# karltan0328/POPE

Measured on AMD Instinct MI355X. Metric: image-pairs/s (DINOv2-S/14 extract+match, 640x480), higher is better.
Workload: dtype f16x3 (fp32 operands split hi+lo into f16, 3 MFMAs per product, fp32 accumulate)

## Files before the change

pope_amd/csrc/attention_f16x3.hip:

```cpp
#include "attention_common.h"
#include "kernels.h"
#include <type_traits>

namespace {
using namespace pope_attn;

typedef __attribute__((address_space(3))) s16x4* lds_s16x4_ptr;

constexpr int WAVES = 8;
constexpr int QB = 32 * WAVES;
constexpr int NT = 64 * WAVES;
constexpr int K_PLANE = KT * KST + 32, V_PLANE = KT * VST + 32;
constexpr size_t X3_ATTN_EPI_BYTES = size_t(32) * WAVES * OST * sizeof(float);

__device__ __forceinline__ void split4(f32x4 v, f16x4& hi, f16x4& lo) { pope_split4(v, hi, lo); }

#ifdef ATTN_STAMPS
__device__ unsigned long long g_attn_dbg[32 * 8];
#define ATTN_STAMP(t, slot)                                                                                     \
    do {                                                                                                        \
        if (blockIdx.x == 300 && tid == 0 && (t) < 32) g_attn_dbg[(t) * 8 + (slot)] = __builtin_readcyclecounter(); \
    } while (0)
#else
#define ATTN_STAMP(t, slot) do {} while (0)
#endif
__device__ unsigned long long g_attn_exact_passes;
constexpr int STAGE_H = 2 * (K_PLANE + V_PLANE);
constexpr size_t X3_ATTN_PIPE_BYTES = size_t(3) * STAGE_H * sizeof(_Float16);
static_assert(X3_ATTN_PIPE_BYTES >= X3_ATTN_EPI_BYTES, "epilogue staging fits the stages");

template <bool OUT_PLANES, bool IN_PLANES, bool DIAG = false>
__global__ __launch_bounds__(NT, 2) void attn_f16x3_pipe_kernel(const float* __restrict__ qkv, float* __restrict__ out,
                                                                  int N, int heads) {
    extern __shared__ __attribute__((aligned(16))) float smem[];
    _Float16* lds = reinterpret_cast<_Float16*>(smem);

    const int tid = threadIdx.x, lane = tid & 63, wave = tid >> 6;
    const int r = lane & 31, h = lane >> 5;
    const Block blk = decode_block(N, heads, QB);
    const int head = blk.head, b = blk.b, q0 = blk.q0;
    const int D = heads * HD, rs = 3 * D;
    const float* base = qkv + size_t(b) * N * rs;
    const int koff = D + head * HD;

    constexpr float QSCALE = 0.125f * 1.44269504088896340736f * (IN_PLANES ? 0.125f * 0.125f : 1.0f);
    f16x8 qh[4], ql[4];
    {
        const int qrow = q0 + wave * 32 + r;
#pragma unroll
        for (int kg = 0; kg < 4; ++kg) {
            f32x4 v0 = {0.f, 0.f, 0.f, 0.f}, v1 = {0.f, 0.f, 0.f, 0.f};
            if (qrow < N) {
                if constexpr (IN_PLANES) {
                    const _Float16* p = reinterpret_cast<const _Float16*>(base) + size_t(qrow) * 2 * rs +
                                        (head * 2 + (kg >> 1)) * 64 + 16 * (kg & 1) + 8 * h;
                    const f16x8 ph = *reinterpret_cast<const f16x8*>(p), pl = *reinterpret_cast<const f16x8*>(p + 32);
#pragma unroll
                    for (int e = 0; e < 4; ++e) {
                        v0[e] = float(ph[e]) + float(pl[e]);
                        v1[e] = float(ph[4 + e]) + float(pl[4 + e]);
                    }
                } else {
                    const float* p = base + size_t(qrow) * rs + head * HD + 16 * kg + 8 * h;
                    v0 = *reinterpret_cast<const f32x4*>(p);
                    v1 = *reinterpret_cast<const f32x4*>(p + 4);
                }
            }
            f16x4 h0, l0, h1, l1;
            split4(v0 * QSCALE, h0, l0);
            split4(v1 * QSCALE, h1, l1);
            qh[kg] = cat(h0, h1);
            ql[kg] = cat(l0, l1);
        }
    }

    const __amdgpu_buffer_rsrc_t rsrc =
        __builtin_amdgcn_make_buffer_rsrc(const_cast<float*>(base), 0, unsigned(N) * unsigned(rs) * 4u, 0x00020000);
    constexpr int RPP = NT / 16, NP = KT / RPP;
    const int srow = tid >> 4, scol = (tid & 15) * 4;
    unsigned kvoff[NP];
#pragma unroll
    for (int i = 0; i < NP; ++i) kvoff[i] = (unsigned(srow + RPP * i) * unsigned(rs) + scol + koff) * 4u;
    const unsigned tile_bytes = unsigned(KT) * unsigned(rs) * 4u, v_delta = unsigned(D) * 4u;
    f32x4 rk[NP], rv[NP];
    auto load_kv = [&](int kt) {
#pragma unroll
        for (int i = 0; i < NP; ++i) {
            rk[i] = __builtin_bit_cast(f32x4, __builtin_amdgcn_raw_buffer_load_b128(rsrc, kvoff[i], kt * tile_bytes, 0));
            rv[i] = __builtin_bit_cast(f32x4, __builtin_amdgcn_raw_buffer_load_b128(rsrc, kvoff[i] + v_delta, kt * tile_bytes, 0));
        }
    };
    f16x4 skh[NP], skl[NP], svh[NP], svl[NP];
    auto split_kv = [&]() {
#pragma unroll
        for (int i = 0; i < NP; ++i) {
            split4(rk[i], skh[i], skl[i]);
            split4(rv[i], svh[i], svl[i]);
        }
    };
    auto write_k_row = [&](int st, int i) {
        _Float16* S = lds + st * STAGE_H;
        *reinterpret_cast<f16x4*>(S + (srow + RPP * i) * KST + scol) = skh[i];
        *reinterpret_cast<f16x4*>(S + K_PLANE + (srow + RPP * i) * KST + scol) = skl[i];
    };
    auto write_v_row = [&](int st, int i) {
        _Float16* S = lds + st * STAGE_H;
        *reinterpret_cast<f16x4*>(S + 2 * K_PLANE + (srow + RPP * i) * VST + scol) = svh[i];
        *reinterpret_cast<f16x4*>(S + 2 * K_PLANE + V_PLANE + (srow + RPP * i) * VST + scol) = svl[i];
    };
    auto write_kv = [&](int st) {
        _Float16* S = lds + st * STAGE_H;
#pragma unroll
        for (int i = 0; i < NP; ++i) {
            *reinterpret_cast<f16x4*>(S + (srow + RPP * i) * KST + scol) = skh[i];
            *reinterpret_cast<f16x4*>(S + K_PLANE + (srow + RPP * i) * KST + scol) = skl[i];
            *reinterpret_cast<f16x4*>(S + 2 * K_PLANE + (srow + RPP * i) * VST + scol) = svh[i];
            *reinterpret_cast<f16x4*>(S + 2 * K_PLANE + V_PLANE + (srow + RPP * i) * VST + scol) = svl[i];
        }
    };

    typedef __attribute__((ext_vector_type(4))) unsigned u32x4;
    u32x4 pa[4] = {}, pb[4] = {};
    const int pkey = tid >> 3, pp = tid & 7;
    const unsigned pl_off = unsigned(pkey) * unsigned(rs) * 4u + unsigned((D >> 5) + head * 2) * 128u + unsigned(pp) * 16u;
    const unsigned pl_vdelta = unsigned(D >> 5) * 128u;
    auto load_planes = [&](int kt, u32x4 (&st)[4]) {
        if (kt * KT >= N) return;
#pragma unroll
        for (int c = 0; c < 4; ++c)
            st[c] = __builtin_amdgcn_raw_buffer_load_b128(rsrc, pl_off + (c >> 1) * pl_vdelta + (c & 1) * 128u, kt * tile_bytes, 0);
    };
    auto write_chunk = [&](int st, int c, const u32x4 (&regs)[4]) {
        _Float16* S = lds + st * STAGE_H + (c < 2 ? 0 : 2 * K_PLANE) + (pp >> 2) * (c < 2 ? K_PLANE : V_PLANE) +
                      pkey * (c < 2 ? KST : VST) + (c & 1) * 32 + (pp & 3) * 8;
        *reinterpret_cast<u32x4*>(S) = regs[c];
    };

    const int v_off = tr_off(lane, h);
    auto vfrag = [&](const _Float16* plane, int u, int s, int dt) {
        const _Float16* p = plane + v_off + (32 * u + 16 * s) * VST + 32 * dt;
        const s16x4 a = __builtin_amdgcn_ds_read_tr16_b64_v4i16((lds_s16x4_ptr)(p));
        const s16x4 c = __builtin_amdgcn_ds_read_tr16_b64_v4i16((lds_s16x4_ptr)(p + 8 * VST));
        return cat(__builtin_bit_cast(f16x4, a), __builtin_bit_cast(f16x4, c));
    };

    f32x16 o0, o1, sb[2][2];
    using P0 = std::integral_constant<int, 0>;
    using P1 = std::integral_constant<int, 1>;
#pragma unroll
    for (int i = 0; i < 16; ++i) { o0[i] = 0.f; o1[i] = 0.f; }
    f32x2 l_run = {0.f, 0.f};
    f32x16 nref;
#pragma unroll
    for (int i = 0; i < 16; ++i) nref[i] = INFINITY;

    struct KFrag { f16x8 k0h, k0l, k1h, k1l; };
    auto read_kfrag = [&](int st, int kg, KFrag& f) {
        const _Float16* kb_h = lds + st * STAGE_H + r * KST + 8 * h + 16 * kg;
        f.k0h = *reinterpret_cast<const f16x8*>(kb_h);
        f.k0l = *reinterpret_cast<const f16x8*>(kb_h + K_PLANE);
        f.k1h = *reinterpret_cast<const f16x8*>(kb_h + 32 * KST);
        f.k1l = *reinterpret_cast<const f16x8*>(kb_h + K_PLANE + 32 * KST);
    };
    auto qk_step = [&](int kg, int j, const KFrag& f, f32x16& d0, f32x16& d1, auto biased) {
        const f32x16 zero = {};
        const f32x16 c_init = decltype(biased)::value ? nref : zero;
        if (j == 0) d0 = mfma_f16(f.k0l, qh[kg], kg == 0 ? c_init : d0);
        if (j == 1) d1 = mfma_f16(f.k1l, qh[kg], kg == 0 ? c_init : d1);
        if (j == 2) d0 = mfma_f16(f.k0h, ql[kg], d0);
        if (j == 3) d1 = mfma_f16(f.k1h, ql[kg], d1);
        if (j == 4) d0 = mfma_f16(f.k0h, qh[kg], d0);
        if (j == 5) d1 = mfma_f16(f.k1h, qh[kg], d1);
    };
    constexpr float LAZY_HEADROOM = 8.0f, LAZY_LIMIT_LOG2 = 15.99f;
    f32x2 sm_ls = {0.f, 0.f};
    auto exact_prepare = [&](const f32x16& c0, const f32x16& c1) __attribute__((always_inline)) {
        float mt = vmax3(c0[0], c1[0], c0[1]);
#pragma unroll
        for (int i = 1; i < 15; ++i) mt = vmax3(mt, c1[i], c0[i + 1]);
        mt = __builtin_fmaxf(mt, c1[15]);
        float ma, mb;
        pope_xor32_pair(mt, ma, mb);
        const float ref_old = -nref[0];
        const float ref_new = __builtin_fmaxf(ref_old, __builtin_fmaxf(ma, mb) - LAZY_HEADROOM);
        const float delta = ref_old - ref_new;
        const float alpha = __builtin_amdgcn_exp2f(delta);
#pragma unroll
        for (int i = 0; i < 16; ++i) nref[i] = -ref_new;
        l_run = l_run * alpha;
#pragma unroll
        for (int e = 0; e < 16; ++e) { o0[e] *= alpha; o1[e] *= alpha; }
        return delta;
    };
    auto exp_pair = [&](int i, f32x16& c0, f32x16& c1, auto biased) __attribute__((always_inline)) {
        f32x16& c = i < 8 ? c0 : c1;
        const int e = 2 * (i & 7);
        if constexpr (decltype(biased)::value) {
            c[e] = __builtin_amdgcn_exp2f(c[e]);
            c[e + 1] = __builtin_amdgcn_exp2f(c[e + 1]);
        } else {
            c[e] = __builtin_amdgcn_exp2f(c[e] + nref[0]);
            c[e + 1] = __builtin_amdgcn_exp2f(c[e + 1] + nref[0]);
        }
        float a0 = sm_ls[0], a1 = sm_ls[1];
        a0 += c[e];
        asm volatile("" : "+v"(a0));
        a1 += c[e + 1];
        asm volatile("" : "+v"(a1));
        sm_ls = f32x2{a0, a1};
    };
    auto softmax_slice = [&](int slot, auto ptag) __attribute__((always_inline)) {
        if (slot == 0) sm_ls = f32x2{0.f, 0.f};
        if (slot % 3 != 2)
            exp_pair((slot / 3) * 2 + slot % 3, sb[decltype(ptag)::value][0], sb[decltype(ptag)::value][1], std::true_type{});
    };
    float la_mt = 0.f;
    auto lookahead_slice = [&](int slot, const f32x16& n0, const f32x16& n1) __attribute__((always_inline)) {
        if (slot == 0) la_mt = vmax3(n0[0], n1[0], n0[1]);
        else if (slot < 15) la_mt = vmax3(la_mt, n1[slot], n0[slot + 1]);
        else if (slot == 15) la_mt = __builtin_fmaxf(la_mt, n1[15]);
    };
    auto advance = [&](f32x16& n0, f32x16& n1) __attribute__((always_inline)) {
        if (__builtin_expect(__builtin_amdgcn_ballot_w64(!(la_mt < LAZY_LIMIT_LOG2)) != 0, 0)) {
            if constexpr (DIAG)
                if (lane == 0) (void)__hip_atomic_fetch_add(&g_attn_exact_passes, 1ull, __ATOMIC_RELAXED, __HIP_MEMORY_SCOPE_AGENT);
            float ma, mb;
            pope_xor32_pair(la_mt, ma, mb);
            const float over = __builtin_fmaxf(__builtin_fmaxf(ma, mb) - LAZY_HEADROOM, 0.f);
            const float delta = -over, alpha = __builtin_amdgcn_exp2f(delta);
            const float nr = nref[0] + delta;
#pragma unroll
            for (int i = 0; i < 16; ++i) nref[i] = nr;
            l_run = l_run * alpha;
#pragma unroll
            for (int e = 0; e < 16; ++e) { o0[e] *= alpha; o1[e] *= alpha; }
#pragma unroll
            for (int i = 0; i < 16; ++i) { n0[i] += delta; n1[i] += delta; }
        }
    };
    auto settle = [&]() __attribute__((always_inline)) { l_run += sm_ls; };
    auto phase1 = [&](int st_next, auto ptag) {
        f32x16& n0 = sb[decltype(ptag)::value ^ 1][0];
        f32x16& n1 = sb[decltype(ptag)::value ^ 1][1];
        KFrag kf[2];
        read_kfrag(st_next, 0, kf[0]);
#pragma unroll
        for (int i = 0; i < 24; ++i) {
            const int kg = i / 6, j = i % 6;
            if (j == 0 && kg < 3) read_kfrag(st_next, kg + 1, kf[(kg + 1) & 1]);
            qk_step(kg, j, kf[kg & 1], n0, n1, std::true_type{});
            softmax_slice(i, ptag);
            __builtin_amdgcn_sched_barrier(0);
        }
    };
    auto softmax_only = [&](auto ptag) {
#pragma unroll
        for (int i = 0; i < 24; ++i) softmax_slice(i, ptag);
    };
    auto split_group = [&](int g, int half, f16x4& hi, f16x4& lo, auto ptag) {
        const int u = g >> 1, s2 = g & 1;
        f32x4 pv4;
#pragma unroll
        for (int e = 0; e < 4; ++e) pv4[e] = sb[decltype(ptag)::value][u][8 * s2 + 4 * half + e];
        split4(pv4, hi, lo);
    };
    auto phase2 = [&](int st, int st_write, auto split_tag, const u32x4 (&pregs)[4], auto ptag, auto look_tag) {
        constexpr bool SPLIT_KV = decltype(split_tag)::value;
        constexpr bool LOOK = decltype(look_tag)::value;
        const _Float16* Vh = lds + st * STAGE_H + 2 * K_PLANE;
        const _Float16* Vl = Vh + V_PLANE;
        f16x4 h0[2], l0[2], h1[2], l1[2];
        f16x8 vh[2][2], vl[2];
        split_group(0, 0, h0[0], l0[0], ptag);
        split_group(0, 1, h1[0], l1[0], ptag);
        vh[0][0] = vfrag(Vh, 0, 0, 0); vl[0] = vfrag(Vl, 0, 0, 0);
        vh[0][1] = vfrag(Vh, 0, 0, 1); vl[1] = vfrag(Vl, 0, 0, 1);
        __builtin_amdgcn_sched_barrier(0);
#pragma unroll
        for (int i = 0; i < 24; ++i) {
            const int g = i / 6, j = i % 6, cur = g & 1, nxt = cur ^ 1;
            const int u = (g + 1) >> 1, s2 = (g + 1) & 1;
            if (j == 0 && g < 3) { vh[nxt][0] = vfrag(Vh, u, s2, 0); vh[nxt][1] = vfrag(Vh, u, s2, 1); }
            const f16x8 ph = cat(h0[cur], h1[cur]), pl = cat(l0[cur], l1[cur]);
            if (j == 0) o0 = mfma_f16(vl[0], ph, o0);
            if (j == 1) o1 = mfma_f16(vl[1], ph, o1);
            if (j == 2) o0 = mfma_f16(vh[cur][0], pl, o0);
            if (j == 3) o1 = mfma_f16(vh[cur][1], pl, o1);
            if (j == 4) o0 = mfma_f16(vh[cur][0], ph, o0);
            if (j == 5) o1 = mfma_f16(vh[cur][1], ph, o1);
            if (j == 2 && g < 3) { vl[0] = vfrag(Vl, u, s2, 0); vl[1] = vfrag(Vl, u, s2, 1); }
            if (g < 3) {
                if (j == 1) split_group(g + 1, 0, h0[nxt], l0[nxt], ptag);
                if (j == 3) split_group(g + 1, 1, h1[nxt], l1[nxt], ptag);
            }
            if (LOOK && i % 3 != 1) lookahead_slice(i - (i + 1) / 3, sb[decltype(ptag)::value ^ 1][0], sb[decltype(ptag)::value ^ 1][1]);
            if (SPLIT_KV && j == 5) {
                if constexpr (IN_PLANES) {
                    write_chunk(st_write, g, pregs);
                } else {
                    const int i2 = g >> 1;
                    if (g & 1) { split4(rv[i2], svh[i2], svl[i2]); write_v_row(st_write, i2); }
                    else { split4(rk[i2], skh[i2], skl[i2]); write_k_row(st_write, i2); }
                }
            }
            __builtin_amdgcn_sched_barrier(0);
        }
    };

    const int nkt = (N + KT - 1) / KT;
    if constexpr (IN_PLANES) {
        load_planes(0, pa);
        load_planes(1, pb);
#pragma unroll
        for (int c = 0; c < 4; ++c) write_chunk(0, c, pa);
        load_planes(2, pa);
    } else {
        load_kv(0);
        split_kv();
        write_kv(0);
        if (nkt > 1) load_kv(1);
    }
    __syncthreads();
    {
        KFrag kf;
#pragma unroll
        for (int kg = 0; kg < 4; ++kg) {
            read_kfrag(0, kg, kf);
#pragma unroll
            for (int j = 0; j < 6; ++j) qk_step(kg, j, kf, sb[0][0], sb[0][1], std::false_type{});
        }
    }
    if (nkt == 1) mask_tail(0, h, N, sb[0][0], sb[0][1]);
    if constexpr (IN_PLANES) {
#pragma unroll
        for (int c = 0; c < 4; ++c) write_chunk(1, c, pb);
        load_planes(3, pb);
    } else if (nkt > 1) {
        split_kv();
        write_kv(1);
        if (nkt > 2) load_kv(2);
    }
    __syncthreads();
    asm volatile("s_nop 15\n\ts_nop 3" : "+v"(sb[0][0]), "+v"(sb[0][1]));
    exact_prepare(sb[0][0], sb[0][1]);
#pragma unroll
    for (int i = 0; i < 16; ++i) { sb[0][0][i] += nref[0]; sb[0][1][i] += nref[0]; }

    int st_cur = 0, st_next = 1, st_write = 2, t = 0;
    auto rotate = [&]() { const int x = st_cur; st_cur = st_next; st_next = st_write; st_write = x; };
    auto steady = [&](u32x4 (&regs)[4], auto ptag) {
        ATTN_STAMP(t, 0);
        phase1(st_next, ptag);
        settle();
        ATTN_STAMP(t, 1);
        phase2(st_cur, st_write, std::true_type{}, regs, ptag, std::true_type{});
        advance(sb[decltype(ptag)::value ^ 1][0], sb[decltype(ptag)::value ^ 1][1]);
        if constexpr (IN_PLANES) load_planes(t + 4, regs);
        else if (t + 3 < nkt) load_kv(t + 3);
        ATTN_STAMP(t, 2);
        __syncthreads();
        ATTN_STAMP(t, 3);
        rotate();
        ++t;
    };
    while (t + 2 < nkt) {
        steady(pa, P0{});
        if (t + 2 < nkt) steady(pb, P1{});
    }
    auto tail = [&](auto ptag) {
        constexpr int P = decltype(ptag)::value;
        using Q = std::integral_constant<int, P ^ 1>;
        if (t + 1 < nkt) {
            phase1(st_next, ptag);
            mask_tail(t + 1, h, N, sb[P ^ 1][0], sb[P ^ 1][1]);
            asm volatile("" : "+v"(sb[P ^ 1][0]), "+v"(sb[P ^ 1][1]));
            settle();
            phase2(st_cur, st_write, std::false_type{}, pa, ptag, std::true_type{});
            advance(sb[P ^ 1][0], sb[P ^ 1][1]);
            rotate();
            ++t;
            softmax_only(Q{});
            settle();
            phase2(st_cur, st_write, std::false_type{}, pa, Q{}, std::false_type{});
        } else {
            softmax_only(ptag);
            settle();
            phase2(st_cur, st_write, std::false_type{}, pa, ptag, std::false_type{});
        }
    };
    if (t & 1) tail(P1{});
    else tail(P0{});
    __syncthreads();

    int tid_e = threadIdx.x;
    asm volatile("" : "+v"(tid_e));
    const int lane_e = tid_e & 63, wave_e = tid_e >> 6, r_e = lane_e & 31, h_e = lane_e >> 5;
    const float l_half = l_run[0] + l_run[1];
    const float inv = (IN_PLANES ? 0.125f : 1.0f) / (l_half + __shfl_xor(l_half, 32));
    float* Os = smem + (wave_e * 32) * OST;
#pragma unroll
    for (int g4 = 0; g4 < 4; ++g4) {
        f32x4 a, c;
#pragma unroll
        for (int e = 0; e < 4; ++e) { a[e] = o0[4 * g4 + e] * inv; c[e] = o1[4 * g4 + e] * inv; }
        *reinterpret_cast<f32x4*>(&Os[r_e * OST + 8 * g4 + 4 * h_e]) = a;
        *reinterpret_cast<f32x4*>(&Os[r_e * OST + 32 + 8 * g4 + 4 * h_e]) = c;
    }
    __builtin_amdgcn_wave_barrier();
#pragma unroll
    for (int i = 0; i < 8; ++i) {
        const int lr = (lane_e >> 4) + 4 * i, c4 = (lane_e & 15) * 4;
        const int qrow = q0 + wave_e * 32 + lr;
        const f32x4 v = *reinterpret_cast<const f32x4*>(&Os[lr * OST + c4]);
        if (qrow < N) {
            if constexpr (OUT_PLANES) {
                f16x4 hi, lo;
                split4(v * 8.0f, hi, lo);
                const int col = head * HD + c4;
                _Float16* o = reinterpret_cast<_Float16*>(out) + (size_t(b) * N + qrow) * 2 * D + pope_planes_col(col);
                __builtin_nontemporal_store(hi, reinterpret_cast<f16x4*>(o));
                __builtin_nontemporal_store(lo, reinterpret_cast<f16x4*>(o + 32));
            } else {
                *reinterpret_cast<f32x4*>(out + (size_t(b) * N + qrow) * D + head * HD + c4) = v;
            }
        }
    }
}

}

static_assert(K_PLANES_ACT_SCALE == 8.0f, "attention planes epilogue scale");

#ifdef ATTN_STAMPS
extern "C" int pope_lab_attn_stamps(unsigned long long* host256) {
    return hipMemcpyFromSymbol(host256, HIP_SYMBOL(g_attn_dbg), sizeof(unsigned long long) * 256) == hipSuccess ? 0 : -1;
}
#endif

int pope_launch_attention_f16x3(const float* qkv, float* out, int B, int N, int heads, hipStream_t stream) {
    unsigned grid;
    if (!args_ok(B, N, heads, QB, 4, 0, 0, qkv, out, &grid)) return POPE_ERR_ARG;
    return pope_launch_lds<attn_f16x3_pipe_kernel<false, false>>(dim3(grid), dim3(NT), X3_ATTN_PIPE_BYTES, stream, qkv, out, N, heads);
}

static int launch_attn_x3_planes(const void* qkv_planes, void* out_planes, int B, int N, int heads, long long* exact_passes_host,
                                 hipStream_t stream) {
    unsigned grid;
    if (!args_ok(B, N, heads, QB, 4, 0, 0, qkv_planes, out_planes, &grid)) return POPE_ERR_ARG;
    const float* qkv = static_cast<const float*>(qkv_planes);
    float* out = static_cast<float*>(out_planes);
    if (!exact_passes_host)
        return pope_launch_lds<attn_f16x3_pipe_kernel<true, true>>(dim3(grid), dim3(NT), X3_ATTN_PIPE_BYTES, stream, qkv, out, N, heads);
    unsigned long long v = 0;
    if (hipMemcpyToSymbol(HIP_SYMBOL(g_attn_exact_passes), &v, sizeof(v)) != hipSuccess) return POPE_ERR_LAUNCH;
    if (pope_launch_lds<attn_f16x3_pipe_kernel<true, true, true>>(dim3(grid), dim3(NT), X3_ATTN_PIPE_BYTES, stream, qkv, out, N, heads) ||
        hipStreamSynchronize(stream) != hipSuccess)
        return POPE_ERR_LAUNCH;
    if (hipMemcpyFromSymbol(&v, HIP_SYMBOL(g_attn_exact_passes), sizeof(v)) != hipSuccess) return POPE_ERR_LAUNCH;
    *exact_passes_host = (long long)v;
    return POPE_OK;
}
int pope_launch_attention_f16x3_planes_io(const void* qkv_planes, void* out_planes, int B, int N, int heads, hipStream_t stream) {
    return launch_attn_x3_planes(qkv_planes, out_planes, B, N, heads, nullptr, stream);
}
int pope_launch_attention_f16x3_planes_io_diag(const void* qkv_planes, void* out_planes, int B, int N, int heads, long long* exact_passes_host,
                                               hipStream_t stream) {
    return exact_passes_host ? launch_attn_x3_planes(qkv_planes, out_planes, B, N, heads, exact_passes_host, stream) : POPE_ERR_ARG;
}
```

pope_amd/csrc/gemm_plain.hip:

```cpp
#include "gemm_core.h"
#include "gemm_routes.h"

namespace {

using gemm_core::EPI_ST;

typedef _Float16 f16x4 __attribute__((ext_vector_type(4)));
typedef _Float16 f16x8 __attribute__((ext_vector_type(8)));
typedef __attribute__((ext_vector_type(4))) unsigned u32x4;
typedef __attribute__((ext_vector_type(2))) unsigned u32x2;
typedef __attribute__((address_space(3))) void* pl_lds_ptr;

constexpr int PL_BM = 256, PL_THREADS = 512;
constexpr float PL_A_SCALE = K_PLANES_ACT_SCALE, PL_W_SCALE = K_PLANES_W_SCALE;
constexpr int pl_stages(int bn) { return bn == 128 ? 3 : 2; }
constexpr size_t pl_lds_bytes(int bn) { return size_t(pl_stages(bn)) * (PL_BM + bn) * 128; }
static_assert(size_t(8) * 32 * EPI_ST * sizeof(float) <= pl_lds_bytes(128), "epilogue staging of the eight waves must fit the stages");

#define PL_FENCE() __builtin_amdgcn_sched_barrier(0x76)

__device__ __forceinline__ f32x4 pl_mfma(f16x8 a, f16x8 b, f32x4 c) { return __builtin_amdgcn_mfma_f32_16x16x32_f16(a, b, c, 0, 0, 0); }

template <int EPI, bool OUT_F16, int NWN, bool X3 = false, int CONV = 0>
__global__ __launch_bounds__(PL_THREADS) void gemm_plain256_kernel(const GemmParams g) {
    constexpr int BN = 64 * NWN, SUB = NWN / 2, ROWS = PL_BM + BN, NST = pl_stages(BN);
    constexpr int STAGE = ROWS * 64;
    extern __shared__ __attribute__((aligned(16))) float smem[];
    _Float16* const lds = reinterpret_cast<_Float16*>(smem);

    const int tid = threadIdx.x, lane = tid & 63;
    const int wave = __builtin_amdgcn_readfirstlane(tid >> 6);
    const int wm = wave / NWN, wn = wave % NWN;
    const int l15 = lane & 15, q4 = lane >> 4;
    const int tiles_n = (g.N + BN - 1) / BN;
    const int tile = xcd_remap(blockIdx.x, gridDim.x);
    constexpr int GROUP_M = X3 ? 1 : 4;
    const int tiles_m = (g.M + PL_BM - 1) / PL_BM, per_group = GROUP_M * tiles_n;
    const int group = tile / per_group, first_m = group * GROUP_M, in_group = tile - group * per_group;
    const int gm = tiles_m - first_m < GROUP_M ? tiles_m - first_m : GROUP_M;
    const int pid_n = in_group / gm, pid_m = first_m + in_group - pid_n * gm;
    const int m0 = pid_m * PL_BM, n0 = pid_n * BN;
    const unsigned lda4 = unsigned(g.lda) * 4u, ldw4 = unsigned(g.ldw) * 4u;
    const unsigned a_rows = CONV == 1 ? unsigned(g.M) + 2u * unsigned(g.conv_wp) + 2u : CONV == 2 ? unsigned(g.conv_s2_in_rows) : unsigned(g.M);
    const __amdgpu_buffer_rsrc_t ra = __builtin_amdgcn_make_buffer_rsrc(const_cast<void*>(g.a_pl), 0, a_rows * lda4, 0x00020000);
    const __amdgpu_buffer_rsrc_t rw = __builtin_amdgcn_make_buffer_rsrc(const_cast<void*>(g.w_pl), 0, unsigned(g.N) * ldw4, 0x00020000);
    const int nk = g.K / 32;

    constexpr int NIW = BN / 64;
    const int r8 = lane >> 3, piece = (lane & 7) ^ r8;
    unsigned va[4], vw[4];
#pragma unroll
    for (int i = 0; i < 4; ++i) {
        unsigned arow = unsigned(m0 + 32 * wave + 8 * i + r8);
        if constexpr (CONV == 2) {
            const unsigned hw = unsigned(g.conv_s2_hpo) * unsigned(g.conv_s2_wpo);
            const unsigned b = arow / hw, rem = arow - b * hw, yo = rem / unsigned(g.conv_s2_wpo), xo = rem - yo * unsigned(g.conv_s2_wpo);
            arow = (b * unsigned(g.conv_s2_hpi) + 2u * yo - 2u) * unsigned(g.conv_wp) + 2u * xo - 2u;
        }
        va[i] = arow * lda4 + unsigned(piece) * 16u;
    }
#pragma unroll
    for (int i = 0; i < NIW; ++i) vw[i] = unsigned(n0 + (BN / 8) * wave + 8 * i + r8) * ldw4 + unsigned(piece) * 16u;
#define PL_DMA2(stage, aoff, woff)                                                                                                \
    do {                                                                                                                         \
        _Float16* S_ = lds + (stage) * STAGE;                                                                                    \
        _Pragma("unroll") for (int i_ = 0; i_ < 4; ++i_)                                                                         \
            __builtin_amdgcn_raw_ptr_buffer_load_lds(ra, (pl_lds_ptr)(S_ + (32 * wave + 8 * i_) * 64), 16, va[i_], (aoff), 0, X3 && CONV == 0 ? 3 : 0); \
        _Pragma("unroll") for (int i_ = 0; i_ < NIW; ++i_)                                                                       \
            __builtin_amdgcn_raw_ptr_buffer_load_lds(rw, (pl_lds_ptr)(S_ + (PL_BM + (BN / 8) * wave + 8 * i_) * 64), 16, vw[i_], (woff), 0, 0); \
    } while (0)
    auto stage_kstep = [&](int stage, int k) {
        if constexpr (CONV == 1) {
            const int chunk = k / 9, tap = k - 9 * chunk, dy = tap / 3, dx = tap - 3 * dy;
            PL_DMA2(stage, unsigned(dy * g.conv_wp + dx) * lda4 + unsigned(chunk) * 128u, unsigned(tap * g.conv_cch + chunk) * 128u);
        } else if constexpr (CONV == 2) {
            const int tap = k / g.conv_cch, chunk = k - tap * g.conv_cch;
            const int ky = g.conv_s2_taps == 9 ? tap / 3 : 1, kx = g.conv_s2_taps == 9 ? tap - 3 * (tap / 3) : 1;
            PL_DMA2(stage, unsigned(ky * g.conv_wp + kx) * lda4 + unsigned(chunk) * 128u, unsigned(k) * 128u);
        } else {
            PL_DMA2(stage, k * 128, k * 128);
        }
    };

    const int a_row = (wm * 64 * SUB + l15) * 64, w_row = (PL_BM + wn * 64 + l15) * 64;
    const int swz0 = 8 * (q4 ^ (l15 & 7)), swz1 = 8 * ((4 + q4) ^ (l15 & 7));

    f32x4 acc[SUB][4][4];
#pragma unroll
    for (int s = 0; s < SUB; ++s)
#pragma unroll
        for (int mi = 0; mi < 4; ++mi)
#pragma unroll
            for (int ni = 0; ni < 4; ++ni) acc[s][mi][ni] = f32x4{0.f, 0.f, 0.f, 0.f};

    stage_kstep(0, 0);
    if (NST == 3 && nk > 1) stage_kstep(1, 1);
    for (int kt = 0; kt < nk; ++kt) {
        if (NST == 3 && kt + 1 < nk) __builtin_amdgcn_s_waitcnt(0x0f70 | (4 + NIW));
        else __builtin_amdgcn_s_waitcnt(0x0f70);
        __syncthreads();
        if (kt + NST - 1 < nk) stage_kstep((kt + NST - 1) % NST, kt + NST - 1);
        const _Float16* S = lds + (kt % NST) * STAGE;
        if constexpr (X3) {
            constexpr int UX = SUB * 4;
            f16x8 wh[4], wl[4], ah[3], al[3];
            auto rd_ax = [&](int r) {
                ah[r % 3] = *reinterpret_cast<const f16x8*>(S + a_row + r * (16 * 64) + swz0);
                al[r % 3] = *reinterpret_cast<const f16x8*>(S + a_row + r * (16 * 64) + swz1);
            };
#pragma unroll
            for (int ni = 0; ni < 4; ++ni) {
                wl[ni] = *reinterpret_cast<const f16x8*>(S + w_row + ni * (16 * 64) + swz1);
                wh[ni] = *reinterpret_cast<const f16x8*>(S + w_row + ni * (16 * 64) + swz0);
            }
            rd_ax(0);
            rd_ax(1);
            PL_FENCE();
#pragma unroll
            for (int r = 0; r < UX; ++r) {
                f32x4(&c)[4] = acc[r >> 2][r & 3];
#pragma unroll
                for (int ni = 0; ni < 4; ++ni) c[ni] = pl_mfma(wl[ni], ah[r % 3], c[ni]);
#pragma unroll
                for (int ni = 0; ni < 4; ++ni) c[ni] = pl_mfma(wh[ni], al[r % 3], c[ni]);
#pragma unroll
                for (int ni = 0; ni < 4; ++ni) c[ni] = pl_mfma(wh[ni], ah[r % 3], c[ni]);
                PL_FENCE();
                if (r + 2 < UX) rd_ax(r + 2);
                PL_FENCE();
            }
        } else {
            constexpr int UPH = SUB * 4, U = 2 * UPH;
            f16x8 wf[2][4], af[4];
            auto rd_a = [&](int u) {
                const int h = u / UPH, r = u % UPH;
                af[u & 3] = *reinterpret_cast<const f16x8*>(S + a_row + r * (16 * 64) + (h ? swz1 : swz0));
            };
            auto rd_w = [&](int h) {
    #pragma unroll
                for (int ni = 0; ni < 4; ++ni) wf[h][ni] = *reinterpret_cast<const f16x8*>(S + w_row + ni * (16 * 64) + (h ? swz1 : swz0));
            };
            rd_w(0);
            rd_a(0);
            rd_a(1);
            rd_a(2);
            PL_FENCE();
    #pragma unroll
            for (int u = 0; u < U; ++u) {
                const int h = u / UPH, r = u % UPH;
    #pragma unroll
                for (int ni = 0; ni < 4; ++ni) acc[r >> 2][r & 3][ni] = pl_mfma(wf[h][ni], af[u & 3], acc[r >> 2][r & 3][ni]);
                PL_FENCE();
                if (u == UPH - 3) rd_w(1);
                if (u + 3 < U) rd_a(u + 3);
                PL_FENCE();
            }
        }
    }

    const unsigned c_row_bytes = unsigned(g.ldc) * 4u;
    const __amdgpu_buffer_rsrc_t rc = __builtin_amdgcn_make_buffer_rsrc(OUT_F16 ? g.c_pl : static_cast<void*>(g.C), 0,
                                                                        unsigned(g.M) * c_row_bytes, 0x00020000);
    const __amdgpu_buffer_rsrc_t rres = __builtin_amdgcn_make_buffer_rsrc(
        const_cast<float*>(EPI == EPI_BIAS_LS_RES ? g.res : g.C), 0,
        EPI == EPI_BIAS_LS_RES ? unsigned(g.res_mod > 0 ? g.res_mod : g.M) * unsigned(g.ldres) * 4u : 0u, 0x00020000);
    auto res_row = [&](unsigned row) -> unsigned { return g.res_mod > 0 ? row % unsigned(g.res_mod) : row; };
    const int ec4 = (lane & 15) * 4, elr = lane >> 4;
    constexpr unsigned DROP = 0xFFFFFF00u;
    constexpr float inv = 1.0f / (PL_A_SCALE * PL_W_SCALE);
    const int col = n0 + wn * 64 + ec4;
    const bool col_ok = col < g.N;
    const int colc = col_ok ? col : 0;
    f32x4 bias = {0.f, 0.f, 0.f, 0.f}, gamma = {0.f, 0.f, 0.f, 0.f};
    if (g.bias) bias = *reinterpret_cast<const f32x4*>(g.bias + colc);
    if constexpr (EPI == EPI_BIAS_LS_RES) {
        gamma = g.gamma ? *reinterpret_cast<const f32x4*>(g.gamma + colc) : f32x4{1.f, 1.f, 1.f, 1.f};
        bias = bias * gamma;
        gamma = gamma * inv;
    }
    [[maybe_unused]] int sq_head = 0, sq_c = 0, sq_row_h = 0;
    [[maybe_unused]] float sq_scale = 1.0f;
    [[maybe_unused]] __amdgpu_buffer_rsrc_t rsq = rres, rmap = rres;
    if constexpr (EPI == EPI_SAM_QKV) {
        const int wcol = n0 + wn * 64;
        const int which = __builtin_amdgcn_readfirstlane((wcol < g.N ? wcol : 0) / g.sam_dim);
        const int rem = colc - which * g.sam_dim;
        sq_head = rem / g.sam_hd;
        sq_c = rem - sq_head * g.sam_hd;
        sq_row_h = which == 2 ? g.sam_dv : g.sam_dq;
        sq_scale = which == 0 ? g.sam_qscale : 1.0f;
        void* dst = which == 0 ? g.sam_q : which == 1 ? g.sam_k : g.sam_v;
        const unsigned bytes = which == 0 ? g.sam_bytes[0] : which == 1 ? g.sam_bytes[1] : g.sam_bytes[2];
        rsq = __builtin_amdgcn_make_buffer_rsrc(dst, 0, bytes, 0x00020000);
        rmap = __builtin_amdgcn_make_buffer_rsrc(const_cast<int*>(g.sam_rowmap), 0, unsigned(g.M) * 4u, 0x00020000);
    }
    [[maybe_unused]] const __amdgpu_buffer_rsrc_t rresp = __builtin_amdgcn_make_buffer_rsrc(
        const_cast<void*>(EPI == EPI_CONV ? g.res_pl : nullptr), 0, EPI == EPI_CONV && g.res_pl ? unsigned(g.M) * unsigned(g.ldres_pl) * 4u : 0u, 0x00020000);
    [[maybe_unused]] const bool col_pad = EPI == EPI_CONV && OUT_F16 && !col_ok && col < g.ldc;
    [[maybe_unused]] float qkv_scale = 1.0f;
    if constexpr (EPI == EPI_QKV_F16) qkv_scale = colc < g.sam_dim ? g.sam_qscale : 1.0f;
    [[maybe_unused]] const int sg_r = lane >> 3, sg_c4 = (lane & 7) * 4, sg_hc = (n0 + wn * 64) / 2 + sg_c4;
    [[maybe_unused]] const bool sg_ok = n0 + wn * 64 < g.N;
    [[maybe_unused]] f32x4 sg_bg = {0.f, 0.f, 0.f, 0.f}, sg_bv = {0.f, 0.f, 0.f, 0.f};
    if constexpr (EPI == EPI_BIAS_SWIGLU) {
        if (g.bias) {
            const float* bp = g.bias + (sg_ok ? n0 + wn * 64 : 0) + sg_c4;
            sg_bg = *reinterpret_cast<const f32x4*>(bp);
            sg_bv = *reinterpret_cast<const f32x4*>(bp + 32);
        }
    }
    __syncthreads();
    float* E = smem + wave * 32 * EPI_ST;
    f32x2 amax = {0.f, 0.f};
    [[maybe_unused]] f32x2 nsum = {0.f, 0.f};
#pragma unroll
    for (int s = 0; s < SUB; ++s) {
        const int m_base = m0 + wm * 64 * SUB + s * 64;
#pragma unroll
        for (int mh = 0; mh < 2; ++mh) {
#pragma unroll
            for (int m2 = 0; m2 < 2; ++m2)
#pragma unroll
                for (int ni = 0; ni < 4; ++ni)
                    *reinterpret_cast<f32x4*>(&E[(m2 * 16 + l15) * EPI_ST + ni * 16 + 4 * q4]) = acc[s][2 * mh + m2][ni];
            const unsigned row0 = unsigned(m_base + mh * 32 + elr);
            [[maybe_unused]] f32x4 res[8];
            if constexpr (EPI == EPI_BIAS_LS_RES) {
#pragma unroll
                for (int i = 0; i < 8; ++i)
                    res[i] = __builtin_bit_cast(f32x4, __builtin_amdgcn_raw_buffer_load_b128(
                                 rres, col_ok ? res_row(row0 + 4 * i) * unsigned(g.ldres) * 4u + unsigned(col) * 4u : DROP, 0, 0));
            }
            [[maybe_unused]] unsigned sq_dest[8];
            if constexpr (EPI == EPI_SAM_QKV) {
#pragma unroll
                for (int i = 0; i < 8; ++i)
                    sq_dest[i] = __builtin_amdgcn_raw_buffer_load_b32(rmap, (row0 + 4 * i) * 4u, 0, 0) + unsigned(sq_head * g.sam_npad);
            }
            if constexpr (EPI == EPI_CONV) {
#pragma unroll
                for (int i = 0; i < 8; ++i) {
                    const unsigned o = (row0 + 4 * i) * unsigned(g.ldres_pl) * 4u + unsigned((col >> 5) * 128 + (col & 31) * 2);
                    const f16x4 rh = __builtin_bit_cast(f16x4, __builtin_amdgcn_raw_buffer_load_b64(rresp, col_ok ? o : DROP, 0, 0));
                    const f16x4 rl = __builtin_bit_cast(f16x4, __builtin_amdgcn_raw_buffer_load_b64(rresp, col_ok ? o + 64u : DROP, 0, 0));
#pragma unroll
                    for (int e = 0; e < 4; ++e) res[i][e] = (float(rh[e]) + float(rl[e])) * (1.0f / PL_A_SCALE);
                }
            }
            __builtin_amdgcn_wave_barrier();
            if constexpr (EPI == EPI_BIAS_SWIGLU) {
                static_assert(EPI != EPI_BIAS_SWIGLU || (X3 && OUT_F16), "the SwiGLU epilogue of this kernel writes planes");
#pragma unroll
                for (int i = 0; i < 4; ++i) {
                    const float* er = &E[(sg_r + 8 * i) * EPI_ST + sg_c4];
                    const f32x4 h = pope_swiglu4(*reinterpret_cast<const f32x4*>(er), *reinterpret_cast<const f32x4*>(er + 32), sg_bg, sg_bv, inv);
                    const unsigned o = sg_ok ? unsigned(m_base + mh * 32 + sg_r + 8 * i) * c_row_bytes + unsigned((sg_hc >> 5) * 128 + (sg_hc & 31) * 2) : DROP;
                    f16x4 hi, lo;
                    pope_amax4x2(amax, h);
                    pope_split4(h * PL_A_SCALE, hi, lo);
                    __builtin_amdgcn_raw_buffer_store_b64(__builtin_bit_cast(u32x2, hi), rc, o, 0, 2);
                    __builtin_amdgcn_raw_buffer_store_b64(__builtin_bit_cast(u32x2, lo), rc, o + 64u, 0, 2);
                }
            } else {
#pragma unroll
            for (int i = 0; i < 8; ++i) {
                f32x4 v = *reinterpret_cast<const f32x4*>(&E[(elr + 4 * i) * EPI_ST + ec4]);
                const unsigned off = (row0 + 4 * i) * c_row_bytes;
                [[maybe_unused]] auto store_planes = [&](f32x4 val) {
                    f16x4 hi, lo;
                    pope_amax4x2(amax, val);
                    pope_split4(val * PL_A_SCALE, hi, lo);
                    const unsigned o = col_ok ? off + unsigned((col >> 5) * 128 + (col & 31) * 2) : DROP;
                    __builtin_amdgcn_raw_buffer_store_b64(__builtin_bit_cast(u32x2, hi), rc, o, 0, 2);
                    __builtin_amdgcn_raw_buffer_store_b64(__builtin_bit_cast(u32x2, lo), rc, o + 64u, 0, 2);
                };
                if constexpr (EPI == EPI_BIAS) {
                    v = v * inv + bias;
                    if constexpr (X3 && OUT_F16) store_planes(v);
                    else __builtin_amdgcn_raw_buffer_store_b128(__builtin_bit_cast(u32x4, v), rc, col_ok ? off + unsigned(col) * 4u : DROP, 0, 2);
                } else if constexpr (EPI == EPI_SAM_QKV) {
                    v = (v * inv + bias) * sq_scale;
                    pope_amax4x2(amax, v);
                    if constexpr (!X3) pope_nan_sum4(nsum, v);
                    const unsigned o = col_ok && row0 + 4 * i < unsigned(g.M) ? (sq_dest[i] * unsigned(sq_row_h) + unsigned(sq_c)) * 2u : DROP;
                    __builtin_amdgcn_raw_buffer_store_b64(__builtin_bit_cast(u32x2, __builtin_convertvector(v, f16x4)), rsq, o, 0, 0);
                } else if constexpr (EPI == EPI_CONV) {
                    v = (v * inv + bias) + res[i];
#pragma unroll
                    for (int e = 0; e < 4; ++e) v[e] = __builtin_fmaxf(v[e], 0.f) + g.act_slope * __builtin_fminf(v[e], 0.f);
                    if constexpr (OUT_F16) {
                        f16x4 hi, lo;
                        pope_amax4x2(amax, v);
                        pope_split4(v * PL_A_SCALE, hi, lo);
                        if (col_pad) { hi = f16x4{0, 0, 0, 0}; lo = f16x4{0, 0, 0, 0}; }
                        const unsigned o = col_ok || col_pad ? off + unsigned((col >> 5) * 128 + (col & 31) * 2) : DROP;
                        __builtin_amdgcn_raw_buffer_store_b64(__builtin_bit_cast(u32x2, hi), rc, o, 0, 2);
                        __builtin_amdgcn_raw_buffer_store_b64(__builtin_bit_cast(u32x2, lo), rc, o + 64u, 0, 2);
                    } else {
                        __builtin_amdgcn_raw_buffer_store_b128(__builtin_bit_cast(u32x4, v), rc, col_ok ? off + unsigned(col) * 4u : DROP, 0, 2);
                    }
                } else if constexpr (EPI == EPI_QKV_F16) {
                    v = (v * inv + bias) * qkv_scale;
                    pope_amax4x2(amax, v);
                    pope_nan_sum4(nsum, v);
                    __builtin_amdgcn_raw_buffer_store_b64(__builtin_bit_cast(u32x2, __builtin_convertvector(v, f16x4)), rc,
                                                          col_ok ? off + unsigned(col) * 2u : DROP, 0, 0);
                } else if constexpr (EPI == EPI_BIAS_GELU) {
                    v = v * inv + bias;
                    const f32x2 g01 = pope_gelu_erf_pair(f32x2{v[0], v[1]}), g23 = pope_gelu_erf_pair(f32x2{v[2], v[3]});
                    v = f32x4{g01[0], g01[1], g23[0], g23[1]};
                    if constexpr (X3 && OUT_F16) {
                        store_planes(v);
                    } else if constexpr (OUT_F16) {
                        pope_amax4x2(amax, v);
                        pope_nan_sum4(nsum, v);
                        const f16x4 hh = __builtin_convertvector(v * PL_A_SCALE, f16x4);
                        __builtin_amdgcn_raw_buffer_store_b64(__builtin_bit_cast(u32x2, hh), rc, col_ok ? off + unsigned(col) * 2u : DROP, 0, 2);
                    } else {
                        __builtin_amdgcn_raw_buffer_store_b128(__builtin_bit_cast(u32x4, v), rc, col_ok ? off + unsigned(col) * 4u : DROP, 0, 2);
                    }
                } else {
                    v = res[i] + v * gamma + bias;
                    __builtin_amdgcn_raw_buffer_store_b128(__builtin_bit_cast(u32x4, v), rc, col_ok ? off + unsigned(col) * 4u : DROP, 0, 0);
                }
            }
            }
            __builtin_amdgcn_wave_barrier();
        }
    }
    if constexpr (EPI == EPI_SAM_QKV || EPI == EPI_QKV_F16)
        pope_range_flag(g.range_flag, g.range_bit, !(__builtin_fmaxf(amax[0], amax[1]) < POPE_F16_OVERFLOW) || (!X3 && pope_nan_seen(nsum)));
    else if constexpr (OUT_F16)
        pope_range_flag(g.range_flag, g.range_bit, !(__builtin_fmaxf(amax[0], amax[1]) * PL_A_SCALE < POPE_F16_OVERFLOW) || (!X3 && pope_nan_seen(nsum)));
}

template <int EPI, bool OUT_F16, int NWN, bool X3 = false, int CONV = 0>
int launch(const GemmParams& g, hipStream_t stream) {
    constexpr int BN = 64 * NWN;
    const int tiles = ((g.M + PL_BM - 1) / PL_BM) * ((g.N + BN - 1) / BN);
    return pope_launch_lds<gemm_plain256_kernel<EPI, OUT_F16, NWN, X3, CONV>>(dim3(tiles), dim3(PL_THREADS), pl_lds_bytes(BN), stream, g);
}

template <int EPI, bool OUT_F16>
int launch_plain_n(const GemmParams& g, hipStream_t stream) {
    return g.N >= 512 ? launch<EPI, OUT_F16, 4>(g, stream) : launch<EPI, OUT_F16, 2>(g, stream);
}

}

bool pope_wide_conv_s2_supported(const GemmParams& g) {
    if (g.plain || !g.a_pl || !g.w_pl || !g.c_pl || g.epilogue != EPI_CONV || g.conv_cch <= 0 || g.nbatch > 1 || g.res_pl) return false;
    if ((g.conv_s2_taps != 9 && g.conv_s2_taps != 1) || g.K != g.conv_s2_taps * 32 * g.conv_cch || g.lda != 32 * g.conv_cch || g.conv_wp < 4) return false;
    if (g.conv_s2_hpo < 3 || g.conv_s2_wpo < 3 || g.conv_s2_hpi < 4 || g.conv_s2_in_rows <= 0 || (g.ldw & 31) || (g.ldc & 31) || g.N > 256) return false;
    if (size_t(g.conv_s2_in_rows) * g.lda * 4 >= (size_t(1) << 32) || size_t(g.N + 256) * g.ldw * 4 >= (size_t(1) << 32) ||
        size_t(g.M + PL_BM) * g.ldc * 4 >= (size_t(1) << 32) - 512)
        return false;
    const int bn = g.N <= 128 ? 128 : 256;
    return size_t((g.M + PL_BM - 1) / PL_BM) * ((g.N + bn - 1) / bn) >= size_t(pope_cu_count());
}

int pope_launch_wide_conv_s2(const GemmParams& g, hipStream_t stream) {
    return g.N <= 128 ? launch<EPI_CONV, true, 2, true, 2>(g, stream) : launch<EPI_CONV, true, 4, true, 2>(g, stream);
}

bool pope_wide_conv_supported(const GemmParams& g) {
    if (g.plain || !g.a_pl || !g.w_pl || g.epilogue != EPI_CONV || g.conv_cch <= 0 || g.nbatch > 1) return false;
    if (g.K != 9 * 32 * g.conv_cch || g.lda != 32 * g.conv_cch || g.conv_wp < 3 || (g.ldw & 31) || (g.ldc & 31)) return false;
    if ((g.c_pl == nullptr) == (g.C == nullptr) || g.N > 256) return false;
    const int bn = g.N <= 128 ? 128 : 256;
    return size_t((g.M + PL_BM - 1) / PL_BM) * ((g.N + bn - 1) / bn) >= size_t(pope_cu_count());
}

int pope_launch_wide_conv(const GemmParams& g, hipStream_t stream) {
    if (size_t(g.M + PL_BM + 2 * g.conv_wp + 2) * g.lda * 4 >= (size_t(1) << 32) || size_t(g.N + 256) * g.ldw * 4 >= (size_t(1) << 32) ||
        size_t(g.M + PL_BM) * g.ldc * 4 >= (size_t(1) << 32) - 512 || (g.res_pl && size_t(g.M + PL_BM) * g.ldres_pl * 4 >= (size_t(1) << 32) - 512))
        return POPE_ERR_ARG;
    if (g.c_pl) return g.N <= 128 ? launch<EPI_CONV, true, 2, true, 1>(g, stream) : launch<EPI_CONV, true, 4, true, 1>(g, stream);
    return g.N <= 128 ? launch<EPI_CONV, false, 2, true, 1>(g, stream) : launch<EPI_CONV, false, 4, true, 1>(g, stream);
}

bool pope_wide_x3_supported(const GemmParams& g) {
    if (g.plain || !g.a_pl || !g.w_pl || !g.c_pl || g.conv_cch > 0 || g.nbatch > 1) return false;
    if (g.epilogue != EPI_BIAS && g.epilogue != EPI_BIAS_GELU && g.epilogue != EPI_BIAS_SWIGLU) return false;
    if (g.N < 512 || (g.N & 63) || g.K < 64 || (g.K & 31) || (g.lda & 31) || (g.ldw & 31) || (g.ldc & 31)) return false;
    return size_t((g.M + PL_BM - 1) / PL_BM) * ((g.N + 255) / 256) >= size_t(4) * pope_cu_count();
}

int pope_launch_wide_x3(const GemmParams& g, hipStream_t stream) {
    if (size_t(g.M + PL_BM) * g.lda * 4 >= (size_t(1) << 32) || size_t(g.N + 256) * g.ldw * 4 >= (size_t(1) << 32) ||
        size_t(g.M + PL_BM) * g.ldc * 4 >= (size_t(1) << 32) - 512)
        return POPE_ERR_ARG;
    if (g.epilogue == EPI_BIAS_SWIGLU) return launch<EPI_BIAS_SWIGLU, true, 4, true>(g, stream);
    return g.epilogue == EPI_BIAS_GELU ? launch<EPI_BIAS_GELU, true, 4, true>(g, stream) : launch<EPI_BIAS, true, 4, true>(g, stream);
}

bool pope_plain256_supported(const GemmParams& g) {
    if (!g.plain || !g.a_pl || !g.w_pl || g.conv_cch > 0 || g.nbatch > 1) return false;
    if (g.M < 2048 || g.N < 256 || (g.N & 63) || g.K < 64 || (g.K & 31) || (g.lda & 31) || (g.ldw & 31)) return false;
    const bool out_f16 = g.c_pl != nullptr;
    switch (g.epilogue) {
        case EPI_BIAS: return !out_f16 && g.C;
        case EPI_BIAS_GELU: return out_f16;
        case EPI_BIAS_LS_RES: return !out_f16 && g.C && g.res;
        case EPI_SAM_QKV: return out_f16;
        case EPI_QKV_F16: return out_f16 && g.sam_dim > 0 && !(g.sam_dim & 63);
    }
    return false;
}

int pope_launch_plain256(const GemmParams& g, hipStream_t stream) {
    if (size_t(g.M + PL_BM) * g.lda * 4 >= (size_t(1) << 32) || size_t(g.N + 256) * g.ldw * 4 >= (size_t(1) << 32) ||
        size_t(g.M + PL_BM) * g.ldc * 4 >= (size_t(1) << 32) - 512 || size_t(g.K) * 4 >= (size_t(1) << 31))
        return POPE_ERR_ARG;
    switch (g.epilogue) {
        case EPI_BIAS: return launch_plain_n<EPI_BIAS, false>(g, stream);
        case EPI_BIAS_GELU: return launch_plain_n<EPI_BIAS_GELU, true>(g, stream);
        case EPI_BIAS_LS_RES: return launch_plain_n<EPI_BIAS_LS_RES, false>(g, stream);
        case EPI_SAM_QKV: return launch_plain_n<EPI_SAM_QKV, true>(g, stream);
        case EPI_QKV_F16: return launch_plain_n<EPI_QKV_F16, true>(g, stream);
    }
    return POPE_ERR_ARG;
}
```

Baseline: 1522.

## Fuse bias/GELU and f16 plane split into plain GEMM epilogue stores

Adds a specialized epilogue path for X3 f16-output bias and bias+GELU GEMMs. It applies bias and GELU directly on accumulator registers, splits the result into hi/lo f16 planes, stages them in LDS and writes them out as full 16-byte row lines. This replaces the generic path that stages fp32 values first and then post-processes them. The attention kernel also gets asm barriers on nref after rescaling, to steer register allocation and scheduling.

```diff
diff --git a/pope_amd/csrc/attention_f16x3.hip b/pope_amd/csrc/attention_f16x3.hip
--- a/pope_amd/csrc/attention_f16x3.hip
+++ b/pope_amd/csrc/attention_f16x3.hip
@@ -187,6 +187,7 @@
         const float alpha = __builtin_amdgcn_exp2f(delta);
 #pragma unroll
         for (int i = 0; i < 16; ++i) nref[i] = -ref_new;
+        asm volatile("" : "+v"(nref));
         l_run = l_run * alpha;
 #pragma unroll
         for (int e = 0; e < 16; ++e) { o0[e] *= alpha; o1[e] *= alpha; }
@@ -231,6 +232,7 @@
             const float nr = nref[0] + delta;
 #pragma unroll
             for (int i = 0; i < 16; ++i) nref[i] = nr;
+            asm volatile("" : "+v"(nref));
             l_run = l_run * alpha;
 #pragma unroll
             for (int e = 0; e < 16; ++e) { o0[e] *= alpha; o1[e] *= alpha; }
diff --git a/pope_amd/csrc/gemm_plain.hip b/pope_amd/csrc/gemm_plain.hip
--- a/pope_amd/csrc/gemm_plain.hip
+++ b/pope_amd/csrc/gemm_plain.hip
@@ -209,6 +209,15 @@
             sg_bv = *reinterpret_cast<const f32x4*>(bp + 32);
         }
     }
+    constexpr bool LINES = X3 && OUT_F16 && CONV == 0 && (EPI == EPI_BIAS || EPI == EPI_BIAS_GELU);
+    [[maybe_unused]] const bool wave_ok = n0 + wn * 64 < g.N;
+    [[maybe_unused]] f32x4 bias_q[4];
+    if constexpr (LINES) {
+#pragma unroll
+        for (int ni = 0; ni < 4; ++ni)
+            bias_q[ni] = g.bias ? *reinterpret_cast<const f32x4*>(g.bias + (wave_ok ? n0 + wn * 64 + ni * 16 + 4 * q4 : 0))
+                                : f32x4{0.f, 0.f, 0.f, 0.f};
+    }
     __syncthreads();
     float* E = smem + wave * 32 * EPI_ST;
     f32x2 amax = {0.f, 0.f};
@@ -218,6 +227,35 @@
         const int m_base = m0 + wm * 64 * SUB + s * 64;
 #pragma unroll
         for (int mh = 0; mh < 2; ++mh) {
+            if constexpr (LINES) {
+#pragma unroll
+                for (int m2 = 0; m2 < 2; ++m2)
+#pragma unroll
+                    for (int ni = 0; ni < 4; ++ni) {
+                        f32x4 v = acc[s][2 * mh + m2][ni] * inv + bias_q[ni];
+                        if constexpr (EPI == EPI_BIAS_GELU) {
+                            const f32x2 g01 = pope_gelu_erf_pair(f32x2{v[0], v[1]}), g23 = pope_gelu_erf_pair(f32x2{v[2], v[3]});
+                            v = f32x4{g01[0], g01[1], g23[0], g23[1]};
+                        }
+                        f16x4 hi, lo;
+                        pope_amax4x2(amax, v);
+                        pope_split4(v * PL_A_SCALE, hi, lo);
+                        _Float16* hp = reinterpret_cast<_Float16*>(E) + (m2 * 16 + l15) * (2 * EPI_ST) + pope_planes_col(ni * 16 + 4 * q4);
+                        *reinterpret_cast<f16x4*>(hp) = hi;
+                        *reinterpret_cast<f16x4*>(hp + 32) = lo;
+                    }
+                __builtin_amdgcn_wave_barrier();
+                if (wave_ok) {
+                    const unsigned o = unsigned(m_base + mh * 32 + (lane >> 4)) * c_row_bytes + unsigned(n0 + wn * 64) * 4u + unsigned(lane & 15) * 16u;
+#pragma unroll
+                    for (int t = 0; t < 8; ++t) {
+                        const f32x4 v = *reinterpret_cast<const f32x4*>(&E[(4 * t + (lane >> 4)) * EPI_ST + (lane & 15) * 4]);
+                        __builtin_amdgcn_raw_buffer_store_b128(__builtin_bit_cast(u32x4, v), rc, o + unsigned(4 * t) * c_row_bytes, 0, 2);
+                    }
+                }
+                __builtin_amdgcn_wave_barrier();
+                continue;
+            }
 #pragma unroll
             for (int m2 = 0; m2 < 2; ++m2)
 #pragma unroll
```

Result: no change. 1534 (median of 6 runs) (+0.8%).
